# mjsargent/gym-miniworld

Hardware: AMD Instinct MI355X
Metric: env-steps/s (80x60 RGB obs) (higher is better)
Workload: dtype f64 sim / f32 render / u8 obs; 1 GPU; maze8192; env_id=MiniWorld-Maze-v0, envs_per_gpu=8192, global_envs=8192, obs=80x60 RGB, domain_rand=False, actions=uniform random over {turn_left, turn_right, move_forward}, counter-based, auto_reset=True, parallelism=env-sharded x1

## Files before the change

gym_miniworld_amd/csrc/mwb_kernels.hip:

```cpp
#include <type_traits>

#include "mwb_internal.h"
#include "mwb_glibc_trig.h"
#include "mwb_lds_layout.h"
#include "mwb_dispatch_map.h"

__device__ __forceinline__ double ref_sin(double x) { return mwb_trig::in_range(x) ? mwb_trig::sin_glibc(x) : sin(x); }
__device__ __forceinline__ double ref_cos(double x) { return mwb_trig::in_range(x) ? mwb_trig::cos_glibc(x) : cos(x); }

__device__ __forceinline__ uint32_t mt_temper(uint32_t y) {
    y ^= (y >> 11);
    y ^= (y << 7) & 0x9d2c5680u;
    y ^= (y << 15) & 0xefc60000u;
    y ^= (y >> 18);
    return y;
}

__device__ __forceinline__ uint32_t mt_mix(uint32_t a, uint32_t b, uint32_t c) {
    uint32_t y = (a & 0x80000000u) | (b & 0x7fffffffu);
    return c ^ (y >> 1) ^ ((y & 1u) ? 0x9908b0dfu : 0u);
}

struct MtSerial {
    uint32_t *key;
// ... 2137 lines not shown
        const float inv = 1.0f / ld[a];
        const float t1 = (lo[a] - lo_[a]) * inv, t2 = (hi[a] - lo_[a]) * inv;
        const float tmin = t1 < t2 ? t1 : t2, tmax = t1 < t2 ? t2 : t1;
        if (tmin > tn) { tn = tmin; face = a * 2 + (ld[a] > 0 ? 0 : 1); }
        if (tmax < tf) tf = tmax;
    }
    if (miss || face <= 0 || !(tn <= tf) || !(tn > 0)) return -1;
    t_out = tn;
    if (face != 1) return 100;
    const float z = fmaf(tn, ld[2], lo_[2]);
    const int n_ch = __float_as_int(fe[FE_FRAME_NCH]);
    int i = (int)floorf((fe[FE_FRAME_HZ] - z) / fe[FE_FRAME_CW]);
    return i < 0 ? 0 : (i >= n_ch ? n_ch - 1 : i);
}
__device__ __forceinline__ bool frame_front_tc(const float *blk, int cell, const float *dv, float &s_, float &t_) {
    const float c = blk[FC_BOX_C], s = blk[FC_BOX_S];
    const float *fe = blk + FC_LIT_BOX;
    const float ld[3] = {fmaf(dv[0], c, -(dv[2] * s)), dv[1], fmaf(dv[0], s, dv[2] * c)};
    const float lo_[3] = {blk[FC_BOX_LO], blk[FC_BOX_LO + 1], blk[FC_BOX_LO + 2]};
    const float tt = (fe[FE_FRAME_SX] - lo_[0]) / ld[0];
    const float y = fmaf(tt, ld[1], lo_[1]), z = fmaf(tt, ld[2], lo_[2]);
    const float z1 = fe[FE_FRAME_HZ] - fe[FE_FRAME_CW] * (float)cell;
    s_ = (z1 - z) / fe[FE_FRAME_CW]; t_ = (y + fe[FE_FRAME_HY]) / (2.0f * fe[FE_FRAME_HY]);
    return ld[0] != 0.0f && tt > 0.0f;
}

struct TexLds { int w, h, n_levels; float sc_s, sc_t; int pad[3]; uint32_t off[MWB_MAX_LEVELS]; };
static_assert(sizeof(TexLds) == sizeof(MwbTexDesc), "TexLds mirrors MwbTexDesc");
static_assert(sizeof(TexLds) == MWB_TEX_LDS_BYTES, "mwb_lds_layout.h sizes the descriptors' region with MWB_TEX_LDS_BYTES");

__device__ __forceinline__ uint32_t footprint_index(uint32_t off, int w, int h, float s, float t, float &a, float &b) {
    float uu = fmaf(s, (float)w, -0.5f), vv = fmaf(t, (float)h, -0.5f);
    float fu = floorf(uu), fv = floorf(vv);
    a = uu - fu; b = vv - fv;
    int i0 = (int)fu, j0 = (int)fv;
    return off + __umul24((uint32_t)(j0 + 1), (uint32_t)(w + 1)) + (uint32_t)(i0 + 1);
}
__device__ __forceinline__ uint4 footprint_load(const uint32_t *__restrict__ texels, uint32_t idx) {
    return *(const uint4 *)((const char *)texels + (size_t)(idx << 4));
}
__device__ __forceinline__ void bilinear_blend(const uint4 fp, float a, float b, float *rgb) {
    const uint32_t t00 = fp.x, t10 = fp.y, t01 = fp.z, t11 = fp.w;
    float w00 = (1.0f - a) * (1.0f - b), w10 = a * (1.0f - b), w01 = (1.0f - a) * b, w11 = a * b;
#pragma unroll
    for (int k = 0; k < 3; k++) {
        float c00 = (float)((t00 >> (8 * k)) & 255u), c10 = (float)((t10 >> (8 * k)) & 255u);
        float c01 = (float)((t01 >> (8 * k)) & 255u), c11 = (float)((t11 >> (8 * k)) & 255u);
        rgb[k] = fmaf(c11, w11, fmaf(c01, w01, fmaf(c10, w10, c00 * w00)));
    }
}

__device__ __forceinline__ void sample_texture(const uint32_t *__restrict__ texels, const TexLds &T, float s, float t, float sx,
                                               float tx, float sy, float ty, bool valid, float *rgb) {
    const int4 dims = *(const int4 *)&T.w;
    const int maxl = dims.z - 1;
    const float fw = (float)dims.x, fh = (float)dims.y;
    const float dsdx = (sx - s) * fw, dtdx = (tx - t) * fh;
    const float dsdy = (sy - s) * fw, dtdy = (ty - t) * fh;
    const float r1 = fmaf(dsdx, dsdx, dtdx * dtdx), r2 = fmaf(dsdy, dsdy, dtdy * dtdy);
    const float rho2 = r1 > r2 ? r1 : r2;
    const float lg = 0.5f * __log2f(fmaxf(rho2, 1.0f));
    const float lambda = (valid && rho2 < INFINITY) ? lg : (float)maxl;
    float ws = s - floorf(s), wt = t - floorf(t);
    ws = (ws >= 0.0f && ws < 1.0f) ? ws : 0.0f;
    wt = (wt >= 0.0f && wt < 1.0f) ? wt : 0.0f;
    const float fl = floorf(lambda);
    int l0 = (int)fl; l0 = l0 > maxl ? maxl : l0;
    const int l1 = l0 + 1 > maxl ? maxl : l0 + 1;
    const float fr = (l0 == maxl) ? 0.0f : lambda - fl;
    float c0[3], c1[3];
    int w0 = dims.x >> l0; w0 = w0 < 1 ? 1 : w0;
    int h0 = dims.y >> l0; h0 = h0 < 1 ? 1 : h0;
    int w1 = dims.x >> l1; w1 = w1 < 1 ? 1 : w1;
    int h1 = dims.y >> l1; h1 = h1 < 1 ? 1 : h1;
    float a0, b0, a1, b1;
    const uint32_t e0 = footprint_index(T.off[l0], w0, h0, ws, wt, a0, b0);
    const uint32_t e1 = footprint_index(T.off[l1], w1, h1, ws, wt, a1, b1);
    const uint4 f0 = footprint_load(texels, e0), f1 = footprint_load(texels, e1);
    bilinear_blend(f0, a0, b0, c0);
    bilinear_blend(f1, a1, b1, c1);
#pragma unroll
    for (int k = 0; k < 3; k++) rgb[k] = fmaf(c1[k] - c0[k], fr, c0[k]);
}

__device__ __forceinline__ bool plane_texcoord(int axis, float plane, float u_org, float u_scale, float sc_t, const float *o,
                                               const float *dv, float &s, float &t) {
    float od = axis == 0 ? dv[0] : axis == 1 ? dv[1] : dv[2];
    float oo = axis == 0 ? o[0] : axis == 1 ? o[1] : o[2];
    float tt = (plane - oo) * __builtin_amdgcn_rcpf(od);
    float px = fmaf(tt, dv[0], o[0]), py = fmaf(tt, dv[1], o[1]), pz = fmaf(tt, dv[2], o[2]);
    float a = axis == 0 ? pz : px;
    float b = axis == 1 ? pz : py;
    s = (a - u_org) * u_scale; t = b * sc_t;
    return od != 0.0f && tt > 0.0f;
}

struct ShapeRuntime {
    __device__ __forceinline__ static int width(const MwbDev &d) { return d.W; }
    __device__ __forceinline__ static int height(const MwbDev &d) { return d.H; }
    __device__ __forceinline__ static int layout(const MwbDev &d) { return d.layout; }
    __device__ __forceinline__ static int want_depth(const MwbDev &d) { return d.want_depth; }
    __device__ __forceinline__ static int debug(const MwbDev &d) { return d.debug_flags; }
    __device__ __forceinline__ static int exp(const MwbDev &d) { return d.exp_flags; }
    __device__ __forceinline__ static bool has_depth(const float *depth) { return depth != nullptr; }
};
template <int W_, int H_, int LAYOUT, bool DEPTH>
struct ShapeFixed {
    __device__ __forceinline__ static constexpr int width(const MwbDev &) { return W_; }
    __device__ __forceinline__ static constexpr int height(const MwbDev &) { return H_; }
    __device__ __forceinline__ static constexpr int layout(const MwbDev &) { return LAYOUT; }
    __device__ __forceinline__ static constexpr int want_depth(const MwbDev &) { return DEPTH ? 1 : 0; }
    __device__ __forceinline__ static constexpr int debug(const MwbDev &) { return 0; }
    __device__ __forceinline__ static constexpr int exp(const MwbDev &) { return 0; }
    __device__ __forceinline__ static constexpr bool has_depth(const float *) { return DEPTH; }
};

template <int NBOX, bool POLY, class SP = ShapeRuntime>
struct RenderCtx {
    const float *rooms, *fc;
    const TexLds *tex;
    const uint32_t *texels;
    uint8_t *fb;
    float *depth;
    Cam cam;
    int n_rooms, cam_room, W, H, layout;
    int depth_stride;
    float cull_cc[1], cull_oc[1][3], zA, zB;
    bool boxes_in_view;
    const MwbMeshDesc *mesh_desc;
    const uint4 *mdesc;
    unsigned long long *mb_slots;
    uint16_t *mb_tasks;
    uint32_t *mb_pix;
    int *mb_count;
    const float4 *mesh_data;
    int exp_flags;
    uint32_t mesh_slots;
    unsigned long long *dbg_counters;
    const uint4 *item_res;
    int part_h_inv;
    __device__ __forceinline__ uint32_t item_boxes(int px, int py) const {
        if (NBOX == 1 || !item_res) return 0xFFFFFFFFu;
        const int item = ((px * 4370) >> 16) * 4 + ((py * part_h_inv) >> 16);
        return item_res[item].z;
    }

    __device__ __forceinline__ static void neighbour_rays_of(const Cam &cam, const float *dc, float *dx, float *dy) {
        const float sx = 2.0f * cam.invW * cam.TW, sy = 2.0f * cam.invH * cam.TH;
#pragma unroll
        for (int k = 0; k < 3; k++) { dx[k] = fmaf(cam.S[k], sx, dc[k]); dy[k] = fmaf(cam.U[k], sy, dc[k]); }
    }
    __device__ __forceinline__ void neighbour_rays(const float *dc, float *dx, float *dy) const { neighbour_rays_of(cam, dc, dx, dy); }

    template <bool PATH>
    __device__ __forceinline__ uint32_t trace_from(int room, const float *dv, float &t_hit, uint32_t &path) const {
        if constexpr (POLY) return trace_rooms_poly<PATH>(rooms, n_rooms, room, cam.eye, dv, t_hit, path);
        else return trace_rooms<PATH>(rooms, n_rooms, room, cam.eye, dv, t_hit, path);
    }
    template <bool PATH>
    __device__ __forceinline__ uint32_t trace(const float *dv, float &t_hit, uint32_t &path) const {
        return trace_from<PATH>(cam_room, dv, t_hit, path);
    }

    template <bool INTERIOR>
    __device__ __forceinline__ void shade_poly(uint32_t key, int first_k, float cx, float cy, float *col) const {
        const uint32_t kind = key & 7u, side = (key >> 3) & 3u;
        if (!INTERIOR) {
            if (kind == KIND_SKY) { col[0] = fc[FC_SKY]; col[1] = fc[FC_SKY + 1]; col[2] = fc[FC_SKY + 2]; return; }
            if (kind == KIND_BOX) {
                const float *lb = fc + FC_LIT_BOX + 3 * ((key >> 3) & 7u) + (NBOX > 1 ? (key >> 6) * FC_BOX_STRIDE : 0u);
                col[0] = lb[0]; col[1] = lb[1]; col[2] = lb[2];
                return;
            }
        }
        const float *r = rooms + __umul24(key >> 6, MWB_POLY_ROOM_WORDS);
        const float height = fabsf(r[PW_HEIGHT]);
        const uint32_t texw = (uint32_t)__float_as_int(r[PW_TEX]);
        const float *ed = r + PW_EDGE0 + __umul24(side, PW_EDGE_WORDS);
        const float4 a = *(const float4 *)ed;
        const float2 n = *(const float2 *)(ed + 4);
        const bool wall = kind == KIND_WALL, floor_ = kind == KIND_FLOOR;
        const uint32_t tex_id = (wall ? texw : floor_ ? (texw >> 8) : (texw >> 16)) & 255u;
        const TexLds &T = tex[tex_id];
        const float sc_s = T.sc_s, sc_t = T.sc_t;
        const float plane = floor_ ? 0.0f : height;
        auto texcoord = [&](const float *dv, float &s, float &t) {
            if (wall) {
                const float den = fmaf(n.y, dv[2], n.x * dv[0]);
                const float tt = fmaf(n.y, a.y - cam.eye[2], n.x * (a.x - cam.eye[0])) * __builtin_amdgcn_rcpf(den);
                const float hx = fmaf(tt, dv[0], cam.eye[0]), hz = fmaf(tt, dv[2], cam.eye[2]), yy = fmaf(tt, dv[1], cam.eye[1]);
                s = fmaf(a.w, hz - a.y, a.z * (hx - a.x)) * sc_s; t = yy * sc_t;
                return den != 0.0f && tt > 0.0f;
            }
            return plane_texcoord(1, plane, 0.0f, sc_s, sc_t, cam.eye, dv, s, t);
        };
        float dc[3], dx[3], dy[3];
        make_ray(cam, cx, cy, dc);
// ... 533 lines not shown
                for (uint32_t bm = NBOX > MWB_MAX_BOXES ? any_boxes & ~mesh_slots : any_boxes; bm; bm &= bm - 1u) {
                    const int bi = __builtin_ctz(bm);
                    const float *fb_ = fc + bi * FC_BOX_STRIDE;
                    const float cc = fb_[FC_CULL_CC];
                    const float b = dv[0] * fb_[FC_CULL_OC] + dv[1] * fb_[FC_CULL_OC + 1] + dv[2] * fb_[FC_CULL_OC + 2];
                    if (((my_boxes >> bi) & 1u) && (cc <= 0.0f || (b > 0.0f && b * b >= dd * cc))) {
                        float tb;
                        int ekind = 0;
                        if constexpr (NBOX > MWB_MAX_BOXES) {
                            const float hxk = __int_as_float(__builtin_amdgcn_readfirstlane(__float_as_int(fb_[FC_BOX_HX])));
                            ekind = hxk == -1.0f ? 1 : hxk == -2.0f ? 2 : 0;
                        }
                        if (ekind == 1) {
                        } else if (ekind == 2) {
                            const int code = trace_frame(fb_, dv, tb);
                            if (code >= 0 && tb < th) { key = KIND_FRAME | ((uint32_t)bi << 3) | ((uint32_t)code << 8); th = tb; }
                        } else {
                            int face = trace_box(fb_, dv, tb);
                            if (face >= 0 && tb < th) { key = MAKE_KEY(KIND_BOX, face, bi); th = tb; }
                        }
                    }
                }
            }
            if (k == 0) { key_s0 = key; t_s0 = th; }
            const bool h0 = (meta & 0xFu) && key == k0, h1 = (meta & 0xF0u) && key == k1;
            const bool h2 = (meta & 0xF00u) && key == k2, h3 = (meta & 0xF000u) && key == k3;
            meta += (h0 ? 1u : 0u) + (h1 ? 0x10u : 0u) + (h2 ? 0x100u : 0u) + (h3 ? 0x1000u : 0u);
            if (!(h0 || h1 || h2 || h3)) {
                if (!(meta & 0xFu)) { k0 = key; meta |= 1u | ((uint32_t)k << 16); }
                else if (!(meta & 0xF0u)) { k1 = key; meta |= 0x10u | ((uint32_t)k << 19); }
                else if (!(meta & 0xF00u)) { k2 = key; meta |= 0x100u | ((uint32_t)k << 22); }
                else if (!(meta & 0xF000u)) { k3 = key; meta |= 0x1000u | ((uint32_t)k << 25); }
                else {
                    float col[3];
                    shade<false>(key, k, cx, cy, col);
                    acc[0] += col[0]; acc[1] += col[1]; acc[2] += col[2];
                }
            }
        }
#pragma unroll 1
        for (int it = 0; it < 4 && (meta & 0xFu); it++) {
            float col[3];
            shade<false>(k0, (meta >> 16) & 7u, cx, cy, col);
            const float cnt = (float)(meta & 0xFu);
#pragma unroll
            for (int q = 0; q < 3; q++) acc[q] += cnt * col[q];
            k0 = k1; k1 = k2; k2 = k3;
            meta = ((meta & 0xFFFFu) >> 4) | ((meta >> 19) << 16);
        }
        write_pixel<false>(px, py, acc, (key_s0 & 7u) != KIND_SKY, t_s0);
    }

    __device__ __forceinline__ void pixel_interior(int px, int py, uint32_t key) const {
        const float cx = (float)px + 0.5f, cy = (float)(H - 1 - py) + 0.5f;
        float col[3];
        shade<true>(key, 0, cx, cy, col);
        float t_s0 = 1.0f;
        if (SP::has_depth(depth)) {
            float dv[3];
            make_ray(cam, cx + c_sample_x[0], cy + c_sample_y[0], dv);
            const uint32_t kind = key & 7u, side = (key >> 3) & 7u;
            if constexpr (POLY) {
                const float *r = rooms + __umul24(key >> 6, MWB_POLY_ROOM_WORDS);
                const float *ed = r + PW_EDGE0 + __umul24(side & 3u, PW_EDGE_WORDS);
                const float den = fmaf(ed[5], dv[2], ed[4] * dv[0]);
                const float num = fmaf(ed[5], ed[1] - cam.eye[2], ed[4] * (ed[0] - cam.eye[0]));
                const float plane = kind == KIND_CEIL ? fabsf(r[PW_HEIGHT]) : 0.0f;
                t_s0 = kind == KIND_WALL ? num / den : (plane - cam.eye[1]) * (1.0f / dv[1]);
                write_pixel<true>(px, py, col, true, t_s0);
                return;
            }
            const float *r = rooms + __umul24(key >> 6, MWB_ROOM_WORDS);
            const float4 rect = *(const float4 *)(r + RW_MINX);
            const bool wall = kind == KIND_WALL;
            const bool is_x = wall && (side == 0u || side == 2u), is_z = wall && (side == 1u || side == 3u);
            const float wall_plane = side == 0u ? rect.y : side == 2u ? rect.x : side == 3u ? rect.w : rect.z;
            const float plane = wall ? wall_plane : (kind == KIND_CEIL ? r[RW_HEIGHT] : 0.0f);
            const float od = is_x ? dv[0] : (is_z ? dv[2] : dv[1]);
            const float oo = is_x ? cam.eye[0] : (is_z ? cam.eye[2] : cam.eye[1]);
            t_s0 = (plane - oo) * (1.0f / od);
        }
        write_pixel<true>(px, py, col, true, t_s0);
    }
};

template <int THREADS>
__device__ __forceinline__ void copy_frame_range(uint8_t *__restrict__ dst, const uint8_t *__restrict__ fb, int begin, int end, int tid,
                                                 uint8_t *__restrict__ dst2 = nullptr) {
    if (((begin | end) & 15) == 0) {
        const uint4 *s4 = (const uint4 *)fb;
        uint4 *d4 = (uint4 *)dst, *e4 = (uint4 *)dst2;
        for (int i = begin / 16 + tid; i < end / 16; i += THREADS) { const uint4 v = s4[i]; d4[i] = v; if (dst2) e4[i] = v; }
    } else if (((begin | end) & 3) == 0) {
        const uint32_t *s1 = (const uint32_t *)fb;
        uint32_t *d1 = (uint32_t *)dst, *e1 = (uint32_t *)dst2;
        for (int i = begin / 4 + tid; i < end / 4; i += THREADS) { const uint32_t v = s1[i]; d1[i] = v; if (dst2) e1[i] = v; }
    } else {
        for (int i = begin + tid; i < end; i += THREADS) { const uint8_t v = fb[i]; dst[i] = v; if (dst2) dst2[i] = v; }
    }
}

template <int THREADS>
__device__ __forceinline__ void stack_put_range(const MwbDev &d, size_t env_base, const uint8_t *__restrict__ src, int b0, int b1, int tid) {
    const size_t dst0 = env_base + (size_t)(d.stk_C - 3) * (d.W * d.H);
    if (d.stk_float) {
        float *o = (float *)d.stk + dst0;
        if (((b0 | b1) & 3) == 0) {
            for (int i = b0 / 4 + tid; i < b1 / 4; i += THREADS) {
                const uint32_t p = ((const uint32_t *)src)[i];
                ((float4 *)o)[i] = make_float4((float)(p & 255u), (float)((p >> 8) & 255u), (float)((p >> 16) & 255u), (float)(p >> 24));
            }
        } else {
            for (int i = b0 + tid; i < b1; i += THREADS) o[i] = (float)src[i];
        }
    } else {
        copy_frame_range<THREADS>((uint8_t *)d.stk + dst0, src, b0, b1, tid);
    }
}

__device__ __forceinline__ float grey_of(uint32_t r, uint32_t g, uint32_t b) {
    return (float)((0.30 * (double)r + 0.59 * (double)g) + 0.11 * (double)b);
}
__device__ __forceinline__ float4 grey_of4(uint32_t r, uint32_t g, uint32_t b) {
    return make_float4(grey_of(r & 255u, g & 255u, b & 255u), grey_of((r >> 8) & 255u, (g >> 8) & 255u, (b >> 8) & 255u),
                       grey_of((r >> 16) & 255u, (g >> 16) & 255u, (b >> 16) & 255u), grey_of(r >> 24, g >> 24, b >> 24));
}
template <int THREADS>
__device__ __noinline__ void grey_put_range(const uint8_t *src, float *dst, float *dst2, int cwh, int plane, int p0, int p1, int vec) {
    const int tid = threadIdx.x;
    int a0 = (p0 + 3) & ~3, a1 = p1 & ~3;
    if (!vec || a0 > a1) { a0 = p1; a1 = p1; }
    for (int i = p0 + tid; i < a0; i += THREADS) {
        const float v = cwh ? grey_of(src[i], src[plane + i], src[2 * plane + i]) : grey_of(src[3 * i], src[3 * i + 1], src[3 * i + 2]);
        dst[i] = v; if (dst2) dst2[i] = v;
    }
    for (int i = a0 / 4 + tid; i < a1 / 4; i += THREADS) {
        float4 v;
        if (cwh) {
            const uint32_t *s1 = (const uint32_t *)src;
            v = grey_of4(s1[i], s1[plane / 4 + i], s1[plane / 2 + i]);
        } else {
            const uint32_t *s1 = (const uint32_t *)src + 3 * i;
            const uint32_t w0 = s1[0], w1 = s1[1], w2 = s1[2];
            v = make_float4(grey_of(w0 & 255u, (w0 >> 8) & 255u, (w0 >> 16) & 255u), grey_of(w0 >> 24, w1 & 255u, (w1 >> 8) & 255u),
                            grey_of((w1 >> 16) & 255u, w1 >> 24, w2 & 255u), grey_of((w2 >> 8) & 255u, (w2 >> 16) & 255u, w2 >> 24));
        }
        ((float4 *)dst)[i] = v; if (dst2) ((float4 *)dst2)[i] = v;
    }
    for (int i = a1 + tid; i < p1; i += THREADS) {
        const float v = cwh ? grey_of(src[i], src[plane + i], src[2 * plane + i]) : grey_of(src[3 * i], src[3 * i + 1], src[3 * i + 2]);
        dst[i] = v; if (dst2) dst2[i] = v;
    }
}
template <int THREADS>
__device__ __forceinline__ void grey_put_env(const MwbDev &d, const int e, const uint8_t *src, int p0, int p1) {
    const int plane = d.W * d.H;
    float *newest = (d.stk && d.stk_cpf == 1) ? (float *)d.stk + ((size_t)e * d.stk_K + d.stk_pos + d.stk_C - 1) * plane : nullptr;
    grey_put_range<THREADS>(src, d.grey + (size_t)e * plane, newest, d.layout == MWB_LAYOUT_CWH, plane, p0, p1, 1);
}

template <int THREADS>
__device__ __noinline__ void keep_frame(uint8_t *frame_keep, const uint8_t *frame, int nbytes, uint8_t *depth_keep, const uint8_t *depth, int zbytes, uint8_t *cached) {
    const int tid = threadIdx.x;
    copy_frame_range<THREADS>(frame_keep, frame, 0, nbytes, tid);
    if (depth_keep) copy_frame_range<THREADS>(depth_keep, depth, 0, zbytes, tid);
    if (tid == 0) *cached = 1;
// ... 89 lines not shown
                    const float *ed = r + PW_EDGE0 + PW_EDGE_WORDS * k;
                    if (!(fmaf(ed[5], cam.eye[2] - ed[1], ed[4] * (cam.eye[0] - ed[0])) >= 0.0f)) in = false;
                }
            } else {
                const float *r = rooms + i * MWB_ROOM_WORDS;
                in = cam.eye[0] >= r[RW_MINX] && cam.eye[0] <= r[RW_MAXX] && cam.eye[2] >= r[RW_MINZ] && cam.eye[2] <= r[RW_MAXZ];
            }
        }
        const unsigned long long m = __ballot(in);
        if (m) { ctx.cam_room = base + (__ffsll((long long)m) - 1); break; }
    }
    const float zn = 0.04f, zf = 100.0f;
    ctx.zA = (zf + zn) / (zf - zn); ctx.zB = (2.0f * zf * zn) / (zf - zn);
    float cull_cc_px[1] = {0.0f};
    if constexpr (NBOX == 1) {
        ctx.cull_cc[0] = uni(fc[FC_CULL_CC]);
        ctx.cull_oc[0][0] = uni(fc[FC_CULL_OC]); ctx.cull_oc[0][1] = uni(fc[FC_CULL_OC + 1]); ctx.cull_oc[0][2] = uni(fc[FC_CULL_OC + 2]);
        cull_cc_px[0] = uni(fc[FC_CULL_CC_PIXEL]);
    }
    ctx.boxes_in_view = __builtin_amdgcn_readfirstlane(__float_as_int(fc[FC_BOX_IN_VIEW])) != 0;
    ctx.item_res = (SP::debug(d) & (1 | 32 | 128)) ? nullptr : item_res;
    ctx.part_h_inv = 65536 / ((H + 3) / 4) + 1;

    const int wave = __builtin_amdgcn_readfirstlane(tid / WAVE), lane = tid % WAVE, n_waves = THREADS / WAVE;
    const int wshift = mwb_coord_bits(W);
    const int wmask = (1 << wshift) - 1;
    const int hshift = mwb_coord_bits(H);
    const int qshift = wshift + hshift, hmask = (1 << hshift) - 1;
    const int skip_max = (SP::debug(d) & 8) || qshift >= 16 ? 0 : (1 << (16 - qshift > 3 ? 3 : 16 - qshift)) - 1;
    uint16_t *queue = queues + wave * QUEUE_CAP;
    uint32_t *iq_key = ikeys + wave * QUEUE_CAP;
    uint16_t *iq_pix = ipix + wave * QUEUE_CAP;
    int q_count = 0, iq_count = 0;
    uint16_t *mqueue = mqueues + wave * MQ_CAP;
    int mq_count = 0;
    const int ci = lane & (TILE_CX - 1), cj = lane / TILE_CX;
    const int n_strips = (W + TILE_CX - 2) / (TILE_CX - 1);
    const int part_h = (H + 3) / 4;
    const bool split_x = SP::layout(d) == MWB_LAYOUT_CWH;
    const int half_strips = (n_strips + 1) / 2;
    const int n_items = part < 0 ? n_strips * 4
                                 : (split_x ? (part == 0 ? half_strips : n_strips - half_strips) * 4 : n_strips * 2);
    (void)n_waves;

    auto box_may_touch = [&](int px, int py, uint32_t boxes ) {
        if (NBOX > 1 && !boxes) return false;
        float dc[3];
        make_ray(cam, (float)px + 0.5f, (float)(H - 1 - py) + 0.5f, dc);
        const float dd = dc[0] * dc[0] + dc[1] * dc[1] + dc[2] * dc[2];
        bool touch = false;
        if constexpr (NBOX == 1) {
            const float b = dc[0] * ctx.cull_oc[0][0] + dc[1] * ctx.cull_oc[0][1] + dc[2] * ctx.cull_oc[0][2];
            touch = cull_cc_px[0] <= 0.0f || (b > 0.0f && b * b >= dd * cull_cc_px[0]);
        } else {
#pragma unroll 1
            for (uint32_t bm = boxes & ((1u << NBOX) - 1u); bm; bm &= bm - 1u) {
                const float *fb_ = fc + __builtin_ctz(bm) * FC_BOX_STRIDE;
                const float ccp = fb_[FC_CULL_CC_PIXEL];
                const float b = dc[0] * fb_[FC_CULL_OC] + dc[1] * fb_[FC_CULL_OC + 1] + dc[2] * fb_[FC_CULL_OC + 2];
                bool t_ = ccp <= 0.0f || (b > 0.0f && b * b >= dd * ccp);
                if constexpr (NBOX > MWB_MAX_BOXES) {
                    if (__builtin_amdgcn_readfirstlane(__float_as_int(fb_[FC_BOX_HX])) == __float_as_int(-1.0f) && t_) {
                        const float *me = fb_ + FC_LIT_BOX;
                        float ld[3];
                        mesh_local_dir(fb_, dc, ld);
                        const float pad = me[FE_MESH_BPAD];
                        const float blo[3] = {-me[FE_MESH_BHX] - pad, -pad, -me[FE_MESH_BHZ] - pad}, bhi[3] = {me[FE_MESH_BHX] + pad, fb_[FC_BOX_SY] + pad, me[FE_MESH_BHZ] + pad};
                        float tn = -INFINITY, tf = INFINITY;
#pragma unroll
                        for (int a = 0; a < 3; a++) {
                            const float inv = 1.0f / ld[a], o_ = fb_[FC_BOX_LO + a];
                            const float t0 = (blo[a] - o_) * inv, t1 = (bhi[a] - o_) * inv;
                            tn = fmaxf(tn, fminf(t0, t1)); tf = fminf(tf, fmaxf(t0, t1));
                        }
                        t_ = tn <= tf && tf > 0.0f;
                    }
                }
                touch = touch || t_;
            }
        }
        return touch;
    };

    auto emit = [&](int px, int py, bool is_pixel, bool interior, uint32_t key, int skip, uint32_t iboxes) {
        bool edge = is_pixel && !interior;
        if constexpr (NBOX > MWB_MAX_BOXES) {
            const bool mesh_px = edge && ctx.boxes_in_view && (iboxes & ctx.mesh_slots) && box_may_touch(px, py, iboxes & ctx.mesh_slots);
            const unsigned long long mm = __ballot(mesh_px);
            if (mesh_px) mqueue[mq_count + __popcll(mm & ((1ull << lane) - 1ull))] = (uint16_t)((skip << qshift) | (py << wshift) | px);
            mq_count += __popcll(mm);
            edge = edge && !mesh_px;
            if (mq_count > MQ_CAP - WAVE) {
                mq_count -= WAVE;
                const int q = mqueue[mq_count + lane];
                if (!(SP::debug(d) & 2)) ctx.pixels_mesh(q & wmask, (q >> wshift) & hmask, q >> qshift, true);
            }
        }
        const unsigned long long em = __ballot(edge);
        if (edge) queue[q_count + __popcll(em & ((1ull << lane) - 1ull))] = (uint16_t)((skip << qshift) | (py << wshift) | px);
        q_count += __popcll(em);
        const unsigned long long im = __ballot(interior);
        if (interior) {
            const int slot = iq_count + __popcll(im & ((1ull << lane) - 1ull));
            iq_key[slot] = key & 0x0FFFFFFFu; iq_pix[slot] = (uint16_t)((py << wshift) | px);
        }
        iq_count += __popcll(im);
        if (iq_count >= WAVE) {
            iq_count -= WAVE;
            const int q = iq_pix[iq_count + lane];
            if (!(SP::debug(d) & 4)) ctx.pixel_interior(q & wmask, q >> wshift, iq_key[iq_count + lane]);
        }
        if (q_count >= WAVE) {
            q_count -= WAVE;
            const int q = queue[q_count + lane];
            if (!(SP::debug(d) & 2)) ctx.pixel_full(q & wmask, (q >> wshift) & hmask, q >> qshift);
        }
    };
    if (!(SP::debug(d) & (1 | 32 | 128))) {
        for (int chunk0 = 0; chunk0 < n_strips; chunk0 += 7) {
            if (wave < 2) {
                const int r = lane >> 3, k = lane & 7, q = wave * 2 + (r >> 2), rr = r & 3;
                const int row0 = q * part_h;
                const int rows = (H - row0) < part_h ? ((H - row0) > 0 ? (H - row0) : 0) : part_h;
                const int ha = rows < 8 ? rows : 8, hb = rows > 8 ? rows - 8 : 0;
                const int crow = row0 + (rr == 0 ? 0 : rr == 1 ? hb : rr == 2 ? ha : rows);
                const int strip = chunk0 + k;
                const int xcol = strip * (TILE_CX - 1) < W ? strip * (TILE_CX - 1) : W;
                float dv[3], th;
                uint32_t path;
                make_ray(cam, (float)xcol, (float)(H - crow), dv);
                uint32_t key = ctx.template trace<true>(dv, th, path);
                const uint32_t kind = key & 7u;
                const bool ok = (kind == KIND_FLOOR || kind == KIND_CEIL || kind == KIND_WALL) && !(path & 0x80000000u);
                const uint32_t path_raw = path;
                if (!ok) { key = 0xF0000000u | (uint32_t)lane; path = (uint32_t)lane; }
                uint32_t nk[8], np[8];
#pragma unroll
                for (int j = 0; j < 8; j++) {
                    const int src = (lane + (j >> 1) * 8 + (j & 1)) & (WAVE - 1);
                    nk[j] = __shfl(key, src); np[j] = __shfl(path, src);
                }
                auto same = [&](int a, int b) { return nk[a] == nk[b] && np[a] == np[b]; };
                const bool top_u = ok && same(0, 1) && same(0, 4) && same(0, 5);
                const bool bot_u = same(2, 3) && same(2, 6) && same(2, 7);
                const bool all_u = top_u && bot_u && same(0, 2);
                int ur0 = 0, ur1 = 0;
                uint32_t ukey = 0;
                if (all_u) { ur1 = rows; ukey = nk[0]; }
                else if (top_u && ha < rows) { ur1 = ha; ukey = nk[0]; }
                else if (bot_u && hb > 0) { ur0 = hb; ur1 = rows; ukey = nk[2]; }
                int common = common_crossings(path_raw, __shfl(path_raw, (lane + 1) & (WAVE - 1)));
                const int c1 = common_crossings(path_raw, __shfl(path_raw, (lane + 24) & (WAVE - 1)));
                const int c2 = common_crossings(path_raw, __shfl(path_raw, (lane + 25) & (WAVE - 1)));
                common = common < c1 ? common : c1; common = common < c2 ? common : c2;
                if ((SP::debug(d) & 8) || ctx.cam_room < 0) common = 0;
                int item_room = ctx.cam_room;
                if (common > 0) {
                    const int r = POLY ? walk_rooms_poly(rooms, ctx.cam_room, cam.eye, dv, common) : walk_rooms(rooms, ctx.cam_room, cam.eye, dv, common);
                    if (r >= 0) item_room = r; else common = 0;
                }
                uint32_t boxes = 0xFFFFFFFFu;
                if (NBOX > 1 && ctx.boxes_in_view) {
                    boxes = 0;
                    const int ix0 = strip * (TILE_CX - 1), iwi = (W - ix0) < (TILE_CX - 1) ? (W - ix0) : (TILE_CX - 1);
                    float c[3], cn;
                    make_ray(cam, (float)ix0 + 0.5f * (float)iwi, (float)(H - row0) - 0.5f * (float)rows, c);
                    cn = __builtin_amdgcn_rsqf(c[0] * c[0] + c[1] * c[1] + c[2] * c[2]);
                    float cos_a = 1.0f;
#pragma unroll
                    for (int j = 0; j < 4; j++) {
                        float e[3];
                        make_ray(cam, (float)(ix0 + ((j & 1) ? iwi : 0)), (float)(H - row0 - ((j & 2) ? rows : 0)), e);
                        const float en = __builtin_amdgcn_rsqf(e[0] * e[0] + e[1] * e[1] + e[2] * e[2]);
                        const float dt = (c[0] * e[0] + c[1] * e[1] + c[2] * e[2]) * cn * en;
                        cos_a = dt < cos_a ? dt : cos_a;
                    }
                    cos_a = cos_a - 0.002f;
                    cos_a = cos_a < 0.0f ? 0.0f : cos_a;
                    const float sin_a = __builtin_sqrtf(1.0f - cos_a * cos_a);
#pragma unroll 1
                    for (int bi = 0; bi < NBOX; bi++) {
                        const float *fb_ = fc + bi * FC_BOX_STRIDE;
                        const float ox = fb_[FC_CULL_OC], oy = fb_[FC_CULL_OC + 1], oz = fb_[FC_CULL_OC + 2], ccp = fb_[FC_CULL_CC_PIXEL];
                        const float oc2 = ox * ox + oy * oy + oz * oz;
                        bool touch = true;
                        if (ccp > 0.0f) {
                            const float idist = __builtin_amdgcn_rsqf(oc2);
                            float sin_b = 1.02f * __builtin_sqrtf(fmaxf(oc2 - ccp, 0.0f)) * idist;
                            sin_b = sin_b > 1.0f ? 1.0f : sin_b;
                            const float cos_b = __builtin_sqrtf(1.0f - sin_b * sin_b);
                            const float cos_t = (c[0] * ox + c[1] * oy + c[2] * oz) * cn * idist;
                            touch = cos_t >= cos_a * cos_b - sin_a * sin_b - 0.02f;
                        }
                        boxes |= touch ? 1u << bi : 0u;
                    }
                }
                if (rr == 0 && k < 7 && strip < n_strips)
                    item_res[strip * 4 + q] = make_uint4(ukey, (uint32_t)(ur0 | (ur1 << 16)), boxes, (uint32_t)((item_room & 0xFFFF) | (common << 16)));
            }
        }
        __syncthreads();
    }

    for (;;) {
        int item = 0;
        if (lane == 0) item = atomicAdd(cam_room_s + 1, 1);
        item = __builtin_amdgcn_readfirstlane(item);
        if (item >= n_items) break;
        if (part >= 0) item = split_x ? item + part * half_strips * 4 : ((item >> 1) << 2) + (item & 1) + 2 * part;
        const int x0 = (item >> 2) * (TILE_CX - 1), row0 = (item & 3) * part_h;
        const int rows = (H - row0) < part_h ? (H - row0) : part_h;
        if (rows <= 0) continue;
        int prow0 = row0, prows = rows;
        int item_skip = 0, item_room = ctx.cam_room;
        uint32_t item_boxes = 0xFFFFFFFFu;
        if (SP::debug(d) & 128) continue;
        if (!(SP::debug(d) & (1 | 32))) {
            const int wi = (W - x0) < (TILE_CX - 1) ? (W - x0) : (TILE_CX - 1);
            const uint4 res = item_res[item];
            const uint32_t ukey = (uint32_t)__builtin_amdgcn_readfirstlane((int)res.x);
            const int urw = __builtin_amdgcn_readfirstlane((int)res.y);
            const int ur0 = urw & 0xFFFF, ur1 = urw >> 16;
            if (NBOX > 1) item_boxes = (uint32_t)__builtin_amdgcn_readfirstlane((int)res.z);
            const int rw = __builtin_amdgcn_readfirstlane((int)res.w);
            item_skip = rw >> 16;
            item_room = (rw & 0xFFFF) == 0xFFFF ? -1 : (rw & 0xFFFF);
            if (ur1 > ur0) {
                if (ur0 == 0 && ur1 == rows) prows = 0;
                else if (ur0 == 0) { prow0 = row0 + ur1; prows = rows - ur1; }
                else prows = ur0;
            }
            const int col = lane & (TILE_CX - 1);
            for (int r0 = ur0; r0 < ur1; r0 += TILE_CY) {
                const int px = x0 + col, py = row0 + r0 + lane / TILE_CX;
                const bool is_pixel = col < wi && py < row0 + ur1;
                bool interior = is_pixel;
                if (interior && ctx.boxes_in_view && box_may_touch(px, py, item_boxes)) interior = false;
                emit(px, py, is_pixel, interior, ukey, 0, item_boxes);
            }
            if (prows <= 0) continue;
        }
        if (SP::debug(d) & 64) continue;
        const int n_pass_i = (prows + 1 + TILE_CY - 1) / TILE_CY;
        uint32_t prev_key = 0, prev_path = 0;
        for (int p = 0; p < n_pass_i; p++) {
            const int crow = prow0 + p * TILE_CY + cj;
            float dv[3], th;
            uint32_t path;
            make_ray(cam, (float)(x0 + ci), (float)(H - crow), dv);
            uint32_t key = ctx.template trace_from<true>(item_room, dv, th, path);
            const uint32_t kind = key & 7u;
            bool ok = (kind == KIND_FLOOR || kind == KIND_CEIL || kind == KIND_WALL) && !(path & 0x80000000u);
            const uint32_t k_br = (uint32_t)__builtin_amdgcn_update_dpp(0, (int)key, 0x101 , 0xf, 0xf, false);
            const uint32_t p_br = (uint32_t)__builtin_amdgcn_update_dpp(0, (int)path, 0x101, 0xf, 0xf, false);
            const uint32_t ck = cj == TILE_CY - 1 ? prev_key : key, cp = cj == TILE_CY - 1 ? prev_path : path;
            const uint32_t k_tl = __shfl(ck, (lane - TILE_CX) & (WAVE - 1)), k_tr = __shfl(ck, (lane - TILE_CX + 1) & (WAVE - 1));
            const uint32_t p_tl = __shfl(cp, (lane - TILE_CX) & (WAVE - 1)), p_tr = __shfl(cp, (lane - TILE_CX + 1) & (WAVE - 1));
            prev_key = key; prev_path = path;
            const int px = x0 + ci, py = crow - 1;
            const bool is_pixel = ci < TILE_CX - 1 && px < W && py >= prow0 && py < prow0 + prows && !(p == 0 && cj == 0);
            bool interior = !(SP::debug(d) & 1) && is_pixel && ok && key == k_br && key == k_tl && key == k_tr &&
                            path == p_br && path == p_tl && path == p_tr;
            if (interior && ctx.boxes_in_view && box_may_touch(px, py, item_boxes)) interior = false;
            int skip = common_crossings4(path, p_br, p_tl, p_tr) + item_skip;
            skip = skip < skip_max ? skip : skip_max;
            emit(px, py, is_pixel, interior, key, skip, item_boxes);
        }
    }
    int *left = cam_room_s + 4;
    if (lane == 0) { left[wave] = iq_count; left[n_waves + wave] = q_count; }
    if constexpr (NBOX > MWB_MAX_BOXES) { if (lane == 0) mleft[wave] = mq_count; }
    __syncthreads();
    if (!(SP::debug(d) & 4)) {
        int g = tid, owner = -1;
#pragma unroll
        for (int w = 0; w < THREADS / WAVE; w++) {
            const int c = left[w];
            if (owner < 0) { if (g < c) owner = w; else g -= c; }
        }
        if (owner >= 0) {
            const int p = ipix[owner * QUEUE_CAP + g];
            ctx.pixel_interior(p & wmask, p >> wshift, ikeys[owner * QUEUE_CAP + g]);
        }
    }
    if (!(SP::debug(d) & 2)) {
        int g = THREADS - 1 - tid, owner = -1;
#pragma unroll
        for (int w = 0; w < THREADS / WAVE; w++) {
            const int c = left[n_waves + w];
            if (owner < 0) { if (g < c) owner = w; else g -= c; }
        }
        if (owner >= 0) {
            const int q = queues[owner * QUEUE_CAP + g];
            ctx.pixel_full(q & wmask, (q >> wshift) & hmask, q >> qshift);
        }
    }
    if constexpr (NBOX > MWB_MAX_BOXES) {
        if (!(SP::debug(d) & 2)) {
            int total = 0;
#pragma unroll
            for (int w = 0; w < THREADS / WAVE; w++) total += mleft[w];
            for (int base = 0; base < total; base += THREADS) {
                int g = base + tid, owner = -1;
#pragma unroll
                for (int w = 0; w < THREADS / WAVE; w++) {
                    const int c = mleft[w];
                    if (owner < 0) { if (g < c) owner = w; else g -= c; }
                }
                if (base + (tid & ~(WAVE - 1)) < total) {
                    const int q = owner >= 0 ? mqueues[owner * MQ_CAP + g] : 0;
                    ctx.pixels_mesh(q & wmask, (q >> wshift) & hmask, q >> qshift, owner >= 0);
                }
            }
        }
    }
    __syncthreads();
    {
        const int nbytes = W * H * 3;
        uint8_t *dst = d.obs + (size_t)e * nbytes;
        uint8_t *keep = (!TILED && !LOOPED && d.frame_cache) ? d.frame_cache + (size_t)e * nbytes : nullptr;
        const uint8_t *zsrc = (keep && SP::want_depth(d)) ? (const uint8_t *)(d.depth + (size_t)e * W * H) : nullptr;
        uint8_t *zkeep = zsrc ? (uint8_t *)(d.depth_cache + (size_t)e * W * H) : nullptr;
        if (TILED) {
            if (SP::layout(d) == MWB_LAYOUT_HWC) {
                uint8_t *big = d.obs + ((size_t)e * SP::width(d) * SP::height(d) + (size_t)ty0 * SP::width(d) + tx0) * 3;
                for (int i = tid; i < H * W * 3; i += THREADS) {
                    const int row = i / (W * 3), col = i - row * (W * 3);
                    big[(size_t)row * SP::width(d) * 3 + col] = fb[i];
                }
            } else {
                uint8_t *big = d.obs + (size_t)e * SP::width(d) * SP::height(d) * 3;
                for (int i = tid; i < H * W * 3; i += THREADS) {
                    const int q = i / (W * H), r = i - q * (W * H), x = r / H, y = r - x * H;
                    big[((size_t)q * SP::width(d) + tx0 + x) * SP::height(d) + ty0 + y] = fb[i];
                }
            }
        } else if (part < 0) {
            copy_frame_range<THREADS>(dst, fb, 0, nbytes, tid, keep);
            if (zsrc) copy_frame_range<THREADS>(zkeep, zsrc, 0, W * H * 4, tid);
        } else if (!split_x) {
            const int mid = 2 * part_h < H ? 2 * part_h : H;
            const int r0 = part ? mid : 0, r1 = part ? H : mid;
            copy_frame_range<THREADS>(dst, fb, r0 * W * 3, r1 * W * 3, tid, keep);
            if (zsrc) copy_frame_range<THREADS>(zkeep, zsrc, r0 * W * 4, r1 * W * 4, tid);
        } else {
            const int midx = half_strips * (TILE_CX - 1) < W ? half_strips * (TILE_CX - 1) : W;
            const int xa = part ? midx : 0, xb = part ? W : midx;
            for (int q = 0; q < 3; q++) copy_frame_range<THREADS>(dst, fb, (q * W + xa) * H, (q * W + xb) * H, tid, keep);
            if (zsrc) {
                const int wx = xb - xa;
                for (int i = tid; i < H * wx; i += THREADS) {
                    const int y = i / wx, o = y * W + xa + (i - y * wx);
// ... 845 lines not shown
```

Before: 15.89 million env-steps/s.

## Software-pipeline interior pixel texture fetches across wave queue flushes

Splits interior-pixel shading into an issue phase, which computes texture coordinates and starts the texel loads, and a finish phase, which does the blend and pixel write. The finish is deferred until the next full wave batch is flushed or the loop ends. The aim is to hide texture memory latency behind the tile-classification work that runs in between. This applies only to the fixed-shape no-depth single-box rectangle-room instantiation, and it costs extra registers to hold the pending tap, which may reduce occupancy.

```diff
diff --git a/gym_miniworld_amd/csrc/mwb_kernels.hip b/gym_miniworld_amd/csrc/mwb_kernels.hip
--- a/gym_miniworld_amd/csrc/mwb_kernels.hip
+++ b/gym_miniworld_amd/csrc/mwb_kernels.hip
@@ -2243,6 +2243,40 @@
 #pragma unroll
     for (int k = 0; k < 3; k++) rgb[k] = fmaf(c1[k] - c0[k], fr, c0[k]);
 }
+struct TexTap { uint4 f0, f1; float a0, b0, a1, b1, fr; };
+__device__ __forceinline__ void sample_issue(const uint32_t *__restrict__ texels, const TexLds &T, float s, float t, float sx,
+                                             float tx, float sy, float ty, bool valid, TexTap &tap) {
+    const int4 dims = *(const int4 *)&T.w;
+    const int maxl = dims.z - 1;
+    const float fw = (float)dims.x, fh = (float)dims.y;
+    const float dsdx = (sx - s) * fw, dtdx = (tx - t) * fh;
+    const float dsdy = (sy - s) * fw, dtdy = (ty - t) * fh;
+    const float r1 = fmaf(dsdx, dsdx, dtdx * dtdx), r2 = fmaf(dsdy, dsdy, dtdy * dtdy);
+    const float rho2 = r1 > r2 ? r1 : r2;
+    const float lg = 0.5f * __log2f(fmaxf(rho2, 1.0f));
+    const float lambda = (valid && rho2 < INFINITY) ? lg : (float)maxl;
+    float ws = s - floorf(s), wt = t - floorf(t);
+    ws = (ws >= 0.0f && ws < 1.0f) ? ws : 0.0f;
+    wt = (wt >= 0.0f && wt < 1.0f) ? wt : 0.0f;
+    const float fl = floorf(lambda);
+    int l0 = (int)fl; l0 = l0 > maxl ? maxl : l0;
+    const int l1 = l0 + 1 > maxl ? maxl : l0 + 1;
+    tap.fr = (l0 == maxl) ? 0.0f : lambda - fl;
+    int w0 = dims.x >> l0; w0 = w0 < 1 ? 1 : w0;
+    int h0 = dims.y >> l0; h0 = h0 < 1 ? 1 : h0;
+    int w1 = dims.x >> l1; w1 = w1 < 1 ? 1 : w1;
+    int h1 = dims.y >> l1; h1 = h1 < 1 ? 1 : h1;
+    const uint32_t e0 = footprint_index(T.off[l0], w0, h0, ws, wt, tap.a0, tap.b0);
+    const uint32_t e1 = footprint_index(T.off[l1], w1, h1, ws, wt, tap.a1, tap.b1);
+    tap.f0 = footprint_load(texels, e0); tap.f1 = footprint_load(texels, e1);
+}
+__device__ __forceinline__ void sample_finish(const TexTap &tap, float *rgb) {
+    float c0[3], c1[3];
+    bilinear_blend(tap.f0, tap.a0, tap.b0, c0);
+    bilinear_blend(tap.f1, tap.a1, tap.b1, c1);
+#pragma unroll
+    for (int k = 0; k < 3; k++) rgb[k] = fmaf(c1[k] - c0[k], tap.fr, c0[k]);
+}
 
 __device__ __forceinline__ bool plane_texcoord(int axis, float plane, float u_org, float u_scale, float sc_t, const float *o,
                                                const float *dv, float &s, float &t) {
@@ -2264,6 +2298,7 @@
     __device__ __forceinline__ static int debug(const MwbDev &d) { return d.debug_flags; }
     __device__ __forceinline__ static int exp(const MwbDev &d) { return d.exp_flags; }
     __device__ __forceinline__ static bool has_depth(const float *depth) { return depth != nullptr; }
+    static constexpr bool pipelined = false;
 };
 template <int W_, int H_, int LAYOUT, bool DEPTH>
 struct ShapeFixed {
@@ -2274,6 +2309,7 @@
     __device__ __forceinline__ static constexpr int debug(const MwbDev &) { return 0; }
     __device__ __forceinline__ static constexpr int exp(const MwbDev &) { return 0; }
     __device__ __forceinline__ static constexpr bool has_depth(const float *) { return DEPTH; }
+    static constexpr bool pipelined = !DEPTH;
 };
 
 template <int NBOX, bool POLY, class SP = ShapeRuntime>
@@ -2973,6 +3009,45 @@
         }
         write_pixel<true>(px, py, col, true, t_s0);
     }
+
+    __device__ __forceinline__ void interior_issue(int px, int py, uint32_t key, TexTap &tap) const {
+        static_assert(!POLY, "shade's rectangle-room set-up");
+        const float cx = (float)px + 0.5f, cy = (float)(H - 1 - py) + 0.5f;
+        const uint32_t kind = key & 7u, side = (key >> 3) & 3u;
+        const float *r = rooms + __umul24(key >> 6, MWB_ROOM_WORDS);
+        const float4 rect = *(const float4 *)(r + RW_MINX);
+        const float height = r[RW_HEIGHT];
+        const uint32_t texw = (uint32_t)__float_as_int(r[RW_TEX]);
+        const float u_org_w = r[RW_SIDE0 + RW_SIDE_WORDS * side + RS_UORG];
+        const bool wall = kind == KIND_WALL, floor_ = kind == KIND_FLOOR;
+        const uint32_t tex_id = (wall ? texw : floor_ ? (texw >> 8) : (texw >> 16)) & 255u;
+        const TexLds &T = tex[tex_id];
+        const bool is_x = wall && !(side & 1u), is_z = wall && (side & 1u);
+        const float wall_plane = side == 0u ? rect.y : side == 2u ? rect.x : side == 3u ? rect.w : rect.z;
+        const int axis = is_x ? 0 : (is_z ? 2 : 1);
+        const float plane = wall ? wall_plane : (floor_ ? 0.0f : height);
+        const float u_org = wall ? u_org_w : 0.0f;
+        const float sc_s = T.sc_s, sc_t = T.sc_t;
+        const float u_scale = (wall && ((texw >> (24 + side)) & 1u)) ? -sc_s : sc_s;
+        float dc[3], dx[3], dy[3];
+        make_ray(cam, cx, cy, dc);
+        neighbour_rays(dc, dx, dy);
+        float s0, t0, s1, t1, s2, t2;
+        plane_texcoord(axis, plane, u_org, u_scale, sc_t, cam.eye, dc, s0, t0);
+        const bool v1 = plane_texcoord(axis, plane, u_org, u_scale, sc_t, cam.eye, dx, s1, t1);
+        const bool v2 = plane_texcoord(axis, plane, u_org, u_scale, sc_t, cam.eye, dy, s2, t2);
+        sample_issue(texels, T, s0, t0, s1, t1, s2, t2, v1 && v2, tap);
+    }
+    __device__ __forceinline__ void interior_finish(int px, int py, uint32_t key, const TexTap &tap) const {
+        static_assert(!POLY && !SP::has_depth(nullptr), "no polygon-room lighting and no depth value here");
+        const uint32_t kind = key & 7u, side = (key >> 3) & 3u;
+        const float *lit = fc + (kind == KIND_WALL ? FC_LIT_WALL + 3 * side : kind == KIND_FLOOR ? FC_LIT_FLOOR : FC_LIT_CEIL);
+        float texel[3], col[3];
+        sample_finish(tap, texel);
+#pragma unroll
+        for (int q = 0; q < 3; q++) col[q] = lit[q] * (texel[q] * (1.0f / 255.0f));
+        write_pixel<true>(px, py, col, true, 1.0f);
+    }
 };
 
 template <int THREADS>
@@ -3228,7 +3303,17 @@
         return touch;
     };
 
-    auto emit = [&](int px, int py, bool is_pixel, bool interior, uint32_t key, int skip, uint32_t iboxes) {
+    constexpr bool PIPE = SP::pipelined && NBOX == 1 && !POLY;
+    TexTap pend_tap = {};
+    uint32_t pend_pix = 0, pend_key = 0;
+    bool pending = false;
+    auto finish_pending = [&]() {
+        if constexpr (PIPE) {
+            if (pending) ctx.interior_finish((int)pend_pix & wmask, (int)pend_pix >> wshift, pend_key, pend_tap);
+            pending = false;
+        }
+    };
+    auto emit =[&](int px, int py, bool is_pixel, bool interior, uint32_t key, int skip, uint32_t iboxes) {
         bool edge = is_pixel && !interior;
         if constexpr (NBOX > MWB_MAX_BOXES) {
             const bool mesh_px = edge && ctx.boxes_in_view && (iboxes & ctx.mesh_slots) && box_may_touch(px, py, iboxes & ctx.mesh_slots);
@@ -3254,7 +3339,14 @@
         if (iq_count >= WAVE) {
             iq_count -= WAVE;
             const int q = iq_pix[iq_count + lane];
-            if (!(SP::debug(d) & 4)) ctx.pixel_interior(q & wmask, q >> wshift, iq_key[iq_count + lane]);
+            if constexpr (PIPE) {
+                finish_pending();
+                pend_pix = (uint32_t)q; pend_key = iq_key[iq_count + lane];
+                ctx.interior_issue(q & wmask, q >> wshift, pend_key, pend_tap);
+                pending = true;
+            } else {
+                if (!(SP::debug(d) & 4)) ctx.pixel_interior(q & wmask, q >> wshift, iq_key[iq_count + lane]);
+            }
         }
         if (q_count >= WAVE) {
             q_count -= WAVE;
@@ -3414,6 +3506,7 @@
         }
     }
     int *left = cam_room_s + 4;
+    if constexpr (PIPE) finish_pending();
     if (lane == 0) { left[wave] = iq_count; left[n_waves + wave] = q_count; }
     if constexpr (NBOX > MWB_MAX_BOXES) { if (lane == 0) mleft[wave] = mq_count; }
     __syncthreads();
```

New measurement: 16.19 million env-steps/s (median of 6 runs). 1.9% higher.
